# Karthik-Ragunath/RAD-NeRF

Measured on AMD Instinct MI355X. Metric: rendered frames/sec @512x512, higher is better.
Workload: dtype f32; 1 GPU; config[1]: inference 512x512, L=16 hash grid T=2^19 F=2 (xyz; ambient/torso grids tiled T=2^16 as shipped), max 16 steps/ray, 25 FPS pose stream, torso pass on; grid=hash19, engine=fused, frames_per_gpu=2122, table_dtype=f32, audio_batch=8, frames_in_flight=1, loop_launch=split, parallelism=frame-parallel x1

## Files before the change

### include/radnerf_fused.h

```cpp
#ifndef RADNERF_FUSED_H
#define RADNERF_FUSED_H

#include "radnerf_hip.h"

#ifdef __cplusplus
extern "C" {
#endif

typedef struct {
    const void *embeddings;
    const int32_t *offsets;
    uint32_t D, L, H;
    float S;
    uint32_t gridtype;
    int dtype;
} rn_grid_t;

typedef struct {
    const float *amb_w0, *amb_w1, *amb_w2;
    const float *sig_w0, *sig_w1, *sig_w2;
    const float *col_w0, *col_w1;
    uint32_t audio_dim, has_eye, ind_dim;
} rn_nerf_weights_t;

size_t rn_nerf_packed_floats(void);
size_t rn_nerf_packed_floats_h16(void);
int rn_nerf_pack_weights_h16(const rn_nerf_weights_t *w, float *packed, rn_stream_t stream);
#define RN_F32_SPLIT 2
size_t rn_nerf_packed_floats_split(void);
int rn_nerf_pack_weights_split(const rn_nerf_weights_t *w, float *packed, rn_stream_t stream);
size_t rn_nerf_bias_floats(void);
int rn_nerf_pack_weights(const rn_nerf_weights_t *w, float *packed, rn_stream_t stream);
int rn_nerf_frame_bias(const rn_nerf_weights_t *w, const float *enc_a, const float *eye, const float *ind_code,
                       float *bias, rn_stream_t stream);
int rn_nerf_frame_bias_batch(const rn_nerf_weights_t *w, const float *enc_a, uint32_t n, const float *eye, const float *ind_code,
                             float *bias, rn_stream_t stream);

int rn_nerf_fused_forward(const float *xyzs, const float *dirs, const float *deltas, uint32_t M,
                          const int32_t *m_dev, const rn_grid_t *grid_xyz, const rn_grid_t *grid_amb,
                          const float *packed, const float *bias, float bound, float *sigmas, float *rgbs,
                          float *ambient, int mlp_dtype, rn_stream_t stream);

#define RN_HEAD_STATE_INTS 64

typedef struct {
    const float *rays_o, *rays_d;
    uint32_t N;
    const float *aabb;
    float min_near;
    const uint8_t *bitfield;
    float bound, dt_gamma;
    uint32_t max_steps, cascade, grid_size;
    float T_thresh;
    float *nears, *fars;
    float *weights_sum, *depth, *image;
    int32_t *rays_alive_a, *rays_alive_b;
    float *rays_t;
    float *xyzs, *dirs, *deltas;
    float *sigmas, *rgbs;
    int32_t *state;
    uint32_t *block_counts;
    int32_t *live_slots;
    uint32_t order_w;
    const int32_t *occ_box;
} rn_head_t;

int rn_head_begin(const rn_head_t *h, rn_stream_t stream);
int rn_head_iterate(const rn_head_t *h, const rn_grid_t *grid_xyz, const rn_grid_t *grid_amb, const float *packed,
                    const float *bias, uint32_t first_iter, uint32_t n_iters, int mlp_dtype, rn_stream_t stream);
#define RN_LOOP_FIRST_MARCHED 1u
#define RN_LOOP_CLOSE_FRAME 2u
#define RN_LOOP_COOP 4u
int rn_head_iterate_ex(const rn_head_t *h, const rn_grid_t *grid_xyz, const rn_grid_t *grid_amb, const float *packed,
                       const float *bias, uint32_t first_iter, uint32_t n_iters, int mlp_dtype, uint32_t flags,
                       rn_stream_t stream);
int rn_frame_begin(const rn_head_t *h, const float *pose, float fx, float fy, float cx, float cy, uint32_t W,
                   rn_stream_t stream);
int rn_head_reschedule(const rn_head_t *h, uint32_t iter_done, uint32_t schedule_N, const int32_t *alive_total,
                       rn_stream_t stream);
#define RN_HEAD_ST_ACTIVE 4
#define RN_HEAD_ST_ITERS 16
#define RN_HEAD_ST_LIVE 17
#define RN_HEAD_ST_SLOTS 18
#define RN_HEAD_ST_UNFINISHED 19
#define RN_HEAD_ST_BARRIER 20
#define RN_HEAD_ST_STALLED 22
#define RN_HEAD_ST_HIST 32
int rn_head_check_done(const rn_head_t *h, uint32_t iters_done, rn_stream_t stream);

typedef struct {
    const float *def_w0, *def_w1, *def_w2;
    const float *tor_w0, *tor_w1, *tor_w2;
    uint32_t ind_dim;
} rn_torso_weights_t;

size_t rn_torso_packed_floats(void);
int rn_torso_pack_weights(const rn_torso_weights_t *w, float *packed, rn_stream_t stream);
int rn_torso_fused(const float *bg_coords, uint32_t N, const float *density_grid_torso, uint32_t grid_size,
                   float thresh, const float *poses6, const float *ind_code, float torso_shrink,
                   const rn_torso_weights_t *w, const float *packed, const rn_grid_t *grid_torso,
                   const float *bg_in, float *bg_out, float *torso_alpha, float *deform, rn_stream_t stream);

int rn_torso_blend_frame(const float *bg_coords, uint32_t N, const float *density_grid_torso, uint32_t grid_size,
                         float thresh, const float *poses6, const float *ind_code, float torso_shrink,
                         const rn_torso_weights_t *w, const float *packed, const rn_grid_t *grid_torso, const float *bg_in,
                         float *bg_out, float *torso_alpha, float *image, const float *weights_sum, float *depth,
                         const float *nears, const float *fars, uint8_t *image_u8, rn_stream_t stream);

#define RN_TORSO_PLAN_MAX_BYTES 268435456
size_t rn_torso_plan_bytes(uint32_t N, uint32_t n_on);
int rn_torso_plan_build(const float *bg_coords, uint32_t N, const float *density_grid_torso, uint32_t grid_size, float thresh,
                        float torso_shrink, void *plan, size_t plan_bytes, uint32_t *n_on, rn_stream_t stream);
int rn_torso_blend_frame_planned(const void *plan, size_t plan_bytes, uint32_t N, uint32_t n_on, const float *poses6,
                                 const float *ind_code, float torso_shrink, const rn_torso_weights_t *w, const float *packed,
                                 const rn_grid_t *grid_torso, const float *bg_in, float *bg_out, float *torso_alpha,
                                 float *deform, float *image, const float *weights_sum, float *depth, const float *nears,
                                 const float *fars, uint8_t *image_u8, rn_stream_t stream);

int rn_torso_mask(const float *bg_coords, uint32_t N, const float *density_grid_torso, uint32_t grid_size, float thresh,
// ... 104 lines not shown
```

### rad-nerf_amd/build.py

```python
import os
import subprocess
import sys
from concurrent.futures import ThreadPoolExecutor

ROOT = os.path.dirname(os.path.abspath(__file__))
CSRC = os.path.join(ROOT, "csrc")
LIBDIR = os.path.join(ROOT, "lib")
LIB = os.path.join(LIBDIR, "libradnerf_hip.so")
INCLUDE = os.path.join(os.path.dirname(ROOT), "include")

HIPCC = os.environ.get("HIPCC", "/opt/rocm/bin/hipcc")
ARCH = "gfx950"
CXXFLAGS = ["-O3", "-std=c++17", "-fPIC", "-ffp-contract=off", f"--offload-arch={ARCH}", "-Wall",
            "-Wno-unused-function", f"-I{INCLUDE}"]


def _sources():
    return sorted(f for f in os.listdir(CSRC) if f.endswith(".hip"))


def _headers():
    hs = [os.path.join(CSRC, f) for f in os.listdir(CSRC) if f.endswith(".h")]
    hs += [os.path.join(INCLUDE, f) for f in os.listdir(INCLUDE) if f.endswith(".h")]
    return hs


def _stale(target, deps):
    if not os.path.exists(target):
        return True
    t = os.path.getmtime(target)
    return any(os.path.getmtime(d) > t for d in deps)


def _compile(src, force):
    obj = os.path.join(CSRC, src[:-4] + ".o")
    path = os.path.join(CSRC, src)
    if force or _stale(obj, [path, __file__] + _headers()):
        cmd = [HIPCC] + CXXFLAGS + ["-c", path, "-o", obj]
        r = subprocess.run(cmd, capture_output=True, text=True)
        if r.returncode != 0:
            raise RuntimeError(f"hipcc failed for {src}:\n{r.stdout}\n{r.stderr}")
        if r.stderr.strip():
            sys.stderr.write(r.stderr)
    return obj


BINDINGS_SRC = os.path.join(CSRC, "bindings", "radnerf_pybind.cpp")
BINDINGS_DIR = os.path.join(LIBDIR, "pybind")
BINDINGS_MODULES = ("_raymarching_face", "_gridencoder", "_shencoder", "_freqencoder")


def build_bindings(force=False, verbose=False):
    import shutil
    import sysconfig
    import torch
    from torch.utils import cpp_extension as ce
    os.makedirs(BINDINGS_DIR, exist_ok=True)
    suffix = sysconfig.get_config_var("EXT_SUFFIX")
    first = os.path.join(BINDINGS_DIR, BINDINGS_MODULES[0] + suffix)
    if force or _stale(first, [BINDINGS_SRC, __file__, LIB] + _headers()):
        tlib = os.path.join(os.path.dirname(torch.__file__), "lib")
        cmd = ["g++", "-O2", "-std=c++17", "-fPIC", "-shared", "-D__HIP_PLATFORM_AMD__=1", "-DUSE_ROCM=1",
               f"-D_GLIBCXX_USE_CXX11_ABI={int(torch._C._GLIBCXX_USE_CXX11_ABI)}", "-Wno-deprecated-declarations"]
        cmd += [f"-I{p}" for p in ce.include_paths()] + [f"-I{sysconfig.get_paths()['include']}", "-I/opt/rocm/include", f"-I{INCLUDE}"]
        cmd += [BINDINGS_SRC, "-o", first, f"-L{tlib}", "-ltorch", "-ltorch_python", "-ltorch_cpu", "-lc10", "-lc10_hip",
                f"-L{LIBDIR}", "-lradnerf_hip", f"-Wl,-rpath,{tlib}", "-Wl,-rpath,$ORIGIN/.."]
        r = subprocess.run(cmd, capture_output=True, text=True)
        if r.returncode != 0:
            raise RuntimeError(f"pybind11 binding failed to build:\n{r.stdout[-3000:]}\n{r.stderr[-3000:]}")
        for name in BINDINGS_MODULES[1:]:
            shutil.copyfile(first, os.path.join(BINDINGS_DIR, name + suffix))
    if verbose:
        print(f"built {BINDINGS_DIR}/{{{', '.join(BINDINGS_MODULES)}}}{suffix}")
    return BINDINGS_DIR


def build_all(force=False, verbose=False):
    os.makedirs(LIBDIR, exist_ok=True)
    srcs = _sources()
    with ThreadPoolExecutor(max_workers=min(4, len(srcs))) as ex:
        objs = list(ex.map(lambda s: _compile(s, force), srcs))
    if force or _stale(LIB, objs):
        cmd = [HIPCC, "-shared", "-fPIC", f"--offload-arch={ARCH}", "-o", LIB] + objs
        r = subprocess.run(cmd, capture_output=True, text=True)
        if r.returncode != 0:
            raise RuntimeError(f"link failed:\n{r.stdout}\n{r.stderr}")
    if verbose:
        print(f"built {LIB}")
    return LIB


if __name__ == "__main__":
    build_all(force="--force" in sys.argv, verbose=True)
    if "--no-bindings" not in sys.argv:
        build_bindings(force="--force" in sys.argv, verbose=True)
```

### rad-nerf_amd/csrc/rn_fused.hip

```cpp
#include "rn_nerf_image_dev.h"

namespace rn {

#ifndef RN_FUSED_PAIR_HASHED
#define RN_FUSED_PAIR_HASHED 0
#endif
#ifndef RN_F32_XYZ_GROUP
#define RN_F32_XYZ_GROUP 1
#endif
#ifndef RN_F32_AMB_GROUP
#define RN_F32_AMB_GROUP 2
#endif
constexpr int kXyzGroup = RN_F32_XYZ_GROUP, kAmbGroup = RN_F32_AMB_GROUP;
#ifndef RN_F32_WAVES
#define RN_F32_WAVES 12
#endif
constexpr int kF32Waves = RN_F32_WAVES, kF32Threads = kF32Waves * kWave;
constexpr bool kPairHashed = RN_FUSED_PAIR_HASHED;

constexpr int kLdsFloats = kInferPacked + kBias;

__global__ void __launch_bounds__(256) k_pack_nerf(RawW w, float *__restrict__ packed) {
    const int e = blockIdx.x * 256 + threadIdx.x;
    if (e >= kInferPacked) return;
    packed[e] = nerf_infer_image_elem(w, e);
}

__global__ void __launch_bounds__(kBias) k_frame_bias(RawW w, const float *__restrict__ enc_a,
                                                      const float *__restrict__ eye,
                                                      const float *__restrict__ ind_code, float *__restrict__ bias) {
    const int t = threadIdx.x;
    enc_a += (size_t)blockIdx.x * w.audio_dim;
    bias += (size_t)blockIdx.x * kBias;
    bias[t] = nerf_const_bias(w, enc_a, eye, ind_code, t);
}

#ifdef RN_PHASE_CLOCK
#define RN_PHASE_MARK(i) const uint64_t phase_t##i = wall_clock64()
#define RN_PHASE_STORE()                                                                                        \
    if (p.ambient && lane < 2 && entry + 1 < M) {                                                               \
        p.ambient[2 * (size_t)sample] = (float)(lane ? phase_t3 - phase_t2 : phase_t1 - phase_t0);                \
        p.ambient[2 * (size_t)sample + 1] = (float)(lane ? phase_t4 - phase_t3 : phase_t2 - phase_t1);            \
    }
#else
#define RN_PHASE_MARK(i)
#define RN_PHASE_STORE()
#endif

template <typename TX, typename TW>
__global__ void __launch_bounds__(kF32Threads, kF32Waves / 4) k_nerf_fused(FusedParams p) {
    __shared__ __attribute__((aligned(16))) float lds[kLdsFloats];
    __shared__ LevelPlan plan_x[16], plan_w[16];

    uint32_t M = p.M;
    if (p.m_dev) { const uint32_t d = (uint32_t)*p.m_dev; M = d < M ? d : M; }
    const uint32_t n_tiles = (M + 31u) >> 5;
    if (workgroup_idle(n_tiles, kF32Waves)) return;

    for (int i = threadIdx.x; i < kInferPacked / 4; i += kF32Threads)
        reinterpret_cast<float4 *>(lds)[i] = reinterpret_cast<const float4 *>(p.packed)[i];
    if (threadIdx.x < kBias) lds[kInferPacked + threadIdx.x] = p.bias[threadIdx.x];
    if (threadIdx.x < 16) {
        const int t = threadIdx.x;
        const uint32_t ox = (uint32_t)p.gx.offsets[t], ow = (uint32_t)p.gw.offsets[t];
        plan_x[t] = plan_level<3>(p.gx.lc.scale[t], p.gx.lc.resolution[t], ox, (uint32_t)p.gx.offsets[t + 1] - ox,
                                  p.gx.gridtype, (uint32_t)sizeof(TX) * 2u);
        plan_w[t] = plan_level<2>(p.gw.lc.scale[t], p.gw.lc.resolution[t], ow, (uint32_t)p.gw.offsets[t + 1] - ow,
                                  p.gw.gridtype, (uint32_t)sizeof(TW) * 2u);
    }
    __syncthreads();

    const int lane = threadIdx.x & 63, wave = threadIdx.x >> 6;
    const int j = lane & 31, h = lane >> 5;
    const int lane_off = h * 64 + j * 2;
    const float *bias_amb = lds + kInferPacked, *bias_sig = lds + kInferPacked + 64, *bias_col = lds + kInferPacked + 128;

    const TileSchedule sched(n_tiles, kF32Waves, (uint32_t)wave);
    for (uint32_t tile = sched.first; tile < sched.end; tile += sched.stride) {
        const uint32_t entry = tile * 32 + j;
        bool live = entry < M;
        uint32_t sample = entry;
        if (p.slots) {
            if (live) sample = (uint32_t)p.slots[entry];
        } else if (live && p.deltas) {
            live = p.deltas[2 * (size_t)sample] != 0.0f;
        }
        if (__ballot(live) == 0ull) continue;

        Acc32 a0, a1, a2;
        RN_PHASE_MARK(0);
        acc_bias(a0, bias_amb, h);
        acc_bias(a2, bias_sig, h);
        {
            float in[3] = {0.0f, 0.0f, 0.0f};
            bool on = live;
            if (live) {
#pragma unroll
                for (int d = 0; d < 3; d++) {
                    in[d] = (p.xyzs[3 * (size_t)sample + d] + p.bound) / (2 * p.bound);
                    on = on && !(in[d] < 0 || in[d] > 1);
                }
            }
            LevelFetch<TX, 3, 2> f[kXyzGroup];
#pragma unroll 1
            for (int r = 0; r < 8; r += kXyzGroup) {
                if (on) {
#pragma unroll
                    for (int i = 0; i < kXyzGroup; i++)
                        issue_planned<TX, 3, 2, kPairHashed, false>(static_cast<const TX *>(p.gx.table), plan_x[2 * (r + i) + h], in, f[i]);
                }
#pragma unroll
                for (int i = 0; i < kXyzGroup; i++) {
                    float f0 = 0.0f, f1 = 0.0f;
                    if (on) {
                        TX res[2];
                        TX dummy[1];
                        blend_level<TX, 3, 2, false>(f[i], 0.0f, res, dummy);
                        f0 = to_f<TX>(res[0]);
                        f1 = to_f<TX>(res[1]);
                    }
                    step32(a0, lds + OFF_A0, 2 * (r + i), lane_off, f0);
                    step32(a2, lds + OFF_S0, 2 * (r + i), lane_off, f0);
                    step32(a0, lds + OFF_A0, 2 * (r + i) + 1, lane_off, f1);
                    step32(a2, lds + OFF_S0, 2 * (r + i) + 1, lane_off, f1);
                }
            }
        }

        RN_PHASE_MARK(1);
        acc_relu(a0);
        acc_zero(a1);
        layer_from_acc(a1, a0, lds + OFF_A1, lane_off);
        acc_relu(a1);
        float amb[2];
        valu_out<2>(a1, lds + OFF_A2, h, amb);
        amb[0] = tanhf(amb[0]);
        amb[1] = tanhf(amb[1]);
        if (p.ambient && live && h == 0) {
            p.ambient[2 * (size_t)sample] = amb[0];
            p.ambient[2 * (size_t)sample + 1] = amb[1];
        }

        RN_PHASE_MARK(2);
        {
            float in[2] = {(amb[0] + 1.0f) / 2.0f, (amb[1] + 1.0f) / 2.0f};
            const bool on = live && !(in[0] < 0 || in[0] > 1 || in[1] < 0 || in[1] > 1);
            LevelFetch<TW, 2, 2> f[kAmbGroup];
#pragma unroll 1
            for (int r = 0; r < 8; r += kAmbGroup) {
                if (on) {
#pragma unroll
                    for (int i = 0; i < kAmbGroup; i++)
                        issue_planned<TW, 2, 2, kPairHashed, false>(static_cast<const TW *>(p.gw.table), plan_w[2 * (r + i) + h], in, f[i]);
                }
#pragma unroll
                for (int i = 0; i < kAmbGroup; i++) {
                    float f0 = 0.0f, f1 = 0.0f;
                    if (on) {
                        TW res[2];
                        TW dummy[1];
                        blend_level<TW, 2, 2, false>(f[i], 0.0f, res, dummy);
                        f0 = to_f<TW>(res[0]);
                        f1 = to_f<TW>(res[1]);
                    }
                    step32(a2, lds + OFF_S0, 16 + 2 * (r + i), lane_off, f0);
                    step32(a2, lds + OFF_S0, 16 + 2 * (r + i) + 1, lane_off, f1);
                }
            }
        }

        RN_PHASE_MARK(3);
        acc_relu(a2);
        acc_zero(a1);
        layer_from_acc(a1, a2, lds + OFF_S1, lane_off);
        acc_relu(a1);
        float sigma;
        {
            float raw[1];
            valu_out<1>(a1, lds + IOFF_S2R, h, raw);
            sigma = expf(raw[0]);
        }
        if (!p.rgbs) {
            if (live && h == 0) p.sigmas[sample] = sigma;
            continue;
        }

        acc_bias(a0, bias_col, h);
        {
            float sh[16];
            float dx = 0.0f, dy = 0.0f, dz = 0.0f;
            if (live) {
                dx = p.dirs[3 * (size_t)sample]; dy = p.dirs[3 * (size_t)sample + 1]; dz = p.dirs[3 * (size_t)sample + 2];
            }
            sh_basis<4>(dx, dy, dz, sh);
#pragma unroll
            for (int s = 0; s < 8; s++) {
                const uint32_t m = 0u - (uint32_t)h;
                const uint32_t b = (__float_as_uint(sh[2 * s]) & ~m) | (__float_as_uint(sh[2 * s + 1]) & m);
                step32(a0, lds + IOFF_C0, s, lane_off, __uint_as_float(b));
            }
        }
#pragma unroll
        for (int s = 0; s < 32; s++) step32(a0, lds + IOFF_C0, 8 + s, lane_off, a1.v[s >> 4][s & 15]);
        acc_relu(a0);
        {
            float rgb[3];
            valu_out<3>(a0, lds + IOFF_C1, h, rgb);
            if (live && h == 0) {
                p.sigmas[sample] = sigma;
#pragma unroll
                for (int c = 0; c < 3; c++) p.rgbs[3 * (size_t)sample + c] = 1.0f / (1.0f + expf(-rgb[c]));
            }
        }
        RN_PHASE_MARK(4);
        RN_PHASE_STORE();
    }
}

int check_fused_grid(const rn_grid_t *g, uint32_t D, const char *name) {
    RN_REQUIRE(g && g->embeddings && g->offsets, "%s: null grid", name);
    RN_REQUIRE(g->D == D && g->L == 16, "%s: fused path needs D=%u, L=16 (got D=%u L=%u)", name, D, g->D, g->L);
    RN_REQUIRE(g->gridtype <= 1 && (g->dtype == RN_F32 || g->dtype == RN_F16), "%s: bad gridtype/dtype", name);
    RN_REQUIRE(((uintptr_t)g->embeddings & 7u) == 0, "%s: table must be 8-byte aligned", name);
    return RN_OK;
}
static int check_w(const rn_nerf_weights_t *w) {
    RN_REQUIRE(w && w->amb_w0 && w->amb_w1 && w->amb_w2 && w->sig_w0 && w->sig_w1 && w->sig_w2 && w->col_w0 && w->col_w1,
               "nerf weights: null pointer");
    RN_REQUIRE(w->has_eye <= 1 && w->audio_dim <= 1024 && w->ind_dim <= 1024, "nerf weights: bad dims");
    return RN_OK;
}

template <typename TX, typename TW>
static void launch_fused(const FusedParams &p, hipStream_t s) {
    const uint32_t n_tiles = (p.M + 31u) >> 5;
    uint32_t blocks = div_up(n_tiles, kF32Waves);
    const uint32_t cap = (uint32_t)num_cus();
    if (blocks > cap) blocks = cap;
    RN_LAUNCH_TIMED((k_nerf_fused<TX, TW>), dim3(blocks), dim3(kF32Threads), s, p);
}

int run_fused(const float *xyzs, const float *dirs, const float *deltas, uint32_t M, const int32_t *m_dev, const rn_grid_t *gx,
              const rn_grid_t *gw, const float *packed, const float *bias, float bound, float *sigmas, float *rgbs, float *ambient,
              int mlp_dtype, hipStream_t s, const int32_t *slots) {
    FusedParams p{xyzs, dirs, deltas, M, m_dev, grid_args(gx), grid_args(gw), packed, bias, bound, sigmas, rgbs, ambient, slots};
    if (mlp_dtype == RN_F32_SPLIT) {
        launch_fused_x2(p, gx->dtype, gw->dtype, (uint32_t)num_cus(), s);
    } else if (mlp_dtype == RN_F16) {
        uint32_t blocks = div_up((M + 63u) >> 6, kWavesPerBlock);
        const uint32_t cap = (uint32_t)num_cus();
        launch_fused_h16(p, gx->dtype, gw->dtype, blocks > cap ? cap : blocks, s);
    } else {
        dispatch_grid_dtypes(gx->dtype, gw->dtype, [&](auto tx, auto tw) { launch_fused<decltype(tx), decltype(tw)>(p, s); });
    }
    return RN_OK;
}

}

using namespace rn;

extern "C" {

size_t rn_nerf_packed_floats(void) { return (size_t)kInferPacked; }
size_t rn_nerf_packed_floats_h16(void) { return packed_floats_h16(); }
size_t rn_nerf_packed_floats_split(void) { return packed_floats_x2(); }

int rn_nerf_pack_weights_split(const rn_nerf_weights_t *w, float *packed, rn_stream_t stream) {
    if (int rc = check_w(w)) return rc;
    RN_REQUIRE(packed && ((uintptr_t)packed & 15u) == 0, "nerf_pack_weights_split: packed must be 16-byte aligned");
    launch_pack_nerf_x2(raw_w(w), packed, as_stream(stream));
    return check_launch("nerf_pack_weights_split");
}

int rn_nerf_pack_weights_h16(const rn_nerf_weights_t *w, float *packed, rn_stream_t stream) {
    if (int rc = check_w(w)) return rc;
    RN_REQUIRE(packed && ((uintptr_t)packed & 15u) == 0, "nerf_pack_weights_h16: packed must be 16-byte aligned");
    launch_pack_nerf_h16(raw_w(w), packed, as_stream(stream));
    return check_launch("nerf_pack_weights_h16");
}
size_t rn_nerf_bias_floats(void) { return (size_t)kBias; }

int rn_nerf_pack_weights(const rn_nerf_weights_t *w, float *packed, rn_stream_t stream) {
    if (int rc = check_w(w)) return rc;
    RN_REQUIRE(packed && ((uintptr_t)packed & 15u) == 0, "nerf_pack_weights: packed must be 16-byte aligned");
    hipLaunchKernelGGL(k_pack_nerf, dim3(div_up(kInferPacked, 256)), dim3(256), 0, as_stream(stream), raw_w(w), packed);
    return check_launch("nerf_pack_weights");
}

int rn_nerf_frame_bias(const rn_nerf_weights_t *w, const float *enc_a, const float *eye, const float *ind_code,
                       float *bias, rn_stream_t stream) {
    if (int rc = check_w(w)) return rc;
    RN_REQUIRE(bias, "nerf_frame_bias: null output");
    RN_REQUIRE(enc_a || w->audio_dim == 0, "nerf_frame_bias: enc_a is required");
    RN_REQUIRE(eye || !w->has_eye, "nerf_frame_bias: eye is required when has_eye");
    RN_REQUIRE(ind_code || w->ind_dim == 0, "nerf_frame_bias: ind_code is required when ind_dim > 0");
    hipLaunchKernelGGL(k_frame_bias, dim3(1), dim3(kBias), 0, as_stream(stream), raw_w(w), enc_a, eye, ind_code, bias);
    return check_launch("nerf_frame_bias");
}

int rn_nerf_frame_bias_batch(const rn_nerf_weights_t *w, const float *enc_a, uint32_t n, const float *eye, const float *ind_code,
                             float *bias, rn_stream_t stream) {
    if (n == 0) return RN_OK;
    if (int rc = check_w(w)) return rc;
    RN_REQUIRE(bias && (enc_a || w->audio_dim == 0) && (eye || !w->has_eye) && (ind_code || w->ind_dim == 0),
               "nerf_frame_bias_batch: null pointer");
    hipLaunchKernelGGL(k_frame_bias, dim3(n), dim3(kBias), 0, as_stream(stream), raw_w(w), enc_a, eye, ind_code, bias);
    return check_launch("nerf_frame_bias_batch");
}

int rn_nerf_fused_forward(const float *xyzs, const float *dirs, const float *deltas, uint32_t M, const int32_t *m_dev,
                          const rn_grid_t *grid_xyz, const rn_grid_t *grid_amb, const float *packed, const float *bias,
                          float bound, float *sigmas, float *rgbs, float *ambient, int mlp_dtype, rn_stream_t stream) {
    if (M == 0) return RN_OK;
    RN_REQUIRE(xyzs && packed && bias && sigmas && (dirs || !rgbs), "nerf_fused_forward: null pointer");
    RN_REQUIRE(((uintptr_t)packed & 15u) == 0, "nerf_fused_forward: packed must be 16-byte aligned");
    if (int rc = check_fused_grid(grid_xyz, 3, "nerf_fused_forward(xyz grid)")) return rc;
    if (int rc = check_fused_grid(grid_amb, 2, "nerf_fused_forward(ambient grid)")) return rc;
    RN_REQUIRE(mlp_dtype == RN_F32 || mlp_dtype == RN_F16 || mlp_dtype == RN_F32_SPLIT,
               "nerf_fused_forward: mlp_dtype must be RN_F32, RN_F16 or RN_F32_SPLIT");
    run_fused(xyzs, dirs, deltas, M, m_dev, grid_xyz, grid_amb, packed, bias, bound, sigmas, rgbs, ambient, mlp_dtype,
              as_stream(stream));
    return check_launch("nerf_fused_forward");
}

}
```

### rad-nerf_amd/csrc/rn_fused_dev.h

```cpp
#pragma once

#include "rn_dda_dev.h"
#include "rn_grid_dev.h"
#include "rn_sh_dev.h"
#include "rn_tile32_dev.h"

#include "../../include/radnerf_fused.h"

#ifndef RN_XCD_TILES
#define RN_XCD_TILES 1
#endif
#ifndef RN_TILE_CHUNK
#define RN_TILE_CHUNK 2
#endif

namespace rn {

constexpr int kFusedThreads = 512;
constexpr int kWavesPerBlock = kFusedThreads / kWave;

struct RawW {
    const float *amb_w0, *amb_w1, *amb_w2, *sig_w0, *sig_w1, *sig_w2, *col_w0, *col_w1;
    uint32_t audio_dim, has_eye, ind_dim;
};
inline RawW raw_w(const rn_nerf_weights_t *w) {
    return RawW{w->amb_w0, w->amb_w1, w->amb_w2, w->sig_w0, w->sig_w1, w->sig_w2, w->col_w0, w->col_w1,
                w->audio_dim, w->has_eye, w->ind_dim};
}

struct Acc {
    f32x16 v[2][2];
};

__device__ __forceinline__ void acc_zero(Acc &a) {
#pragma unroll
    for (int nt = 0; nt < 2; nt++)
#pragma unroll
        for (int rt = 0; rt < 2; rt++)
#pragma unroll
            for (int r = 0; r < 16; r++) a.v[nt][rt][r] = 0.0f;
}

__device__ __forceinline__ void acc_bias(Acc &a, const float *bias64, int h) {
#pragma unroll
    for (int rt = 0; rt < 2; rt++)
#pragma unroll
        for (int g = 0; g < 4; g++) {
            const float4 b = *reinterpret_cast<const float4 *>(bias64 + 32 * rt + 8 * g + 4 * h);
            a.v[0][rt][4 * g + 0] = b.x; a.v[0][rt][4 * g + 1] = b.y; a.v[0][rt][4 * g + 2] = b.z; a.v[0][rt][4 * g + 3] = b.w;
            a.v[1][rt][4 * g + 0] = b.x; a.v[1][rt][4 * g + 1] = b.y; a.v[1][rt][4 * g + 2] = b.z; a.v[1][rt][4 * g + 3] = b.w;
        }
}

__device__ __forceinline__ void acc_relu(Acc &a) {
#pragma unroll
    for (int nt = 0; nt < 2; nt++)
#pragma unroll
        for (int rt = 0; rt < 2; rt++)
#pragma unroll
            for (int r = 0; r < 16; r++) a.v[nt][rt][r] = relu_bits(a.v[nt][rt][r]);
}


template <int NOUT>
__device__ __forceinline__ void valu_out(const Acc &in, const float *wl, int h, float (&part)[2][NOUT]) {
#pragma unroll
    for (int o = 0; o < NOUT; o++) {
        float p0 = 0.0f, p1 = 0.0f;
        const float *wo = wl + (o * 2 + h) * 32;
#pragma unroll
        for (int g = 0; g < 8; g++) {
            const float4 w = *reinterpret_cast<const float4 *>(wo + 4 * g);
            const int rt = g >> 2, r = (g & 3) * 4;
            p0 = __builtin_fmaf(in.v[0][rt][r + 0], w.x, p0); p1 = __builtin_fmaf(in.v[1][rt][r + 0], w.x, p1);
            p0 = __builtin_fmaf(in.v[0][rt][r + 1], w.y, p0); p1 = __builtin_fmaf(in.v[1][rt][r + 1], w.y, p1);
            p0 = __builtin_fmaf(in.v[0][rt][r + 2], w.z, p0); p1 = __builtin_fmaf(in.v[1][rt][r + 2], w.z, p1);
            p0 = __builtin_fmaf(in.v[0][rt][r + 3], w.w, p0); p1 = __builtin_fmaf(in.v[1][rt][r + 3], w.w, p1);
        }
        part[0][o] = p0 + __shfl_xor(p0, 32, 64);
        part[1][o] = p1 + __shfl_xor(p1, 32, 64);
    }
}


struct GridArgs {
    const void *table;
    const int32_t *offsets;
    LevelConsts lc;
    uint32_t gridtype;
};
inline GridArgs grid_args(const rn_grid_t *g) {
    return GridArgs{g->embeddings, g->offsets, make_level_consts(g->L, g->S, g->H), g->gridtype};
}

struct FusedParams {
    const float *xyzs, *dirs, *deltas;
    uint32_t M;
    const int32_t *m_dev;
    GridArgs gx, gw;
    const float *packed, *bias;
    float bound;
    float *sigmas, *rgbs, *ambient;
    const int32_t *slots;
};

struct TileSchedule {
    uint32_t first, end, stride;
    __device__ __forceinline__ TileSchedule(uint32_t n_tiles, uint32_t waves_per_block, uint32_t wave) {
        const uint32_t G = gridDim.x, b = blockIdx.x;
#if RN_XCD_TILES
        if (G >= 8 && (G & 7u) == 0) {
            const uint32_t xcd = b & 7u, local = b >> 3, per_xcd = (n_tiles + 7u) >> 3;
            const uint32_t lo = xcd * per_xcd, hi = lo + per_xcd < n_tiles ? lo + per_xcd : n_tiles;
            constexpr uint32_t C = RN_TILE_CHUNK;
            const uint32_t chunk = (C < waves_per_block && waves_per_block % C == 0) ? C : waves_per_block, B = G >> 3;
            first = lo + ((wave / chunk) * B + local) * chunk + wave % chunk;
            end = lo < hi ? hi : lo;
            stride = B * waves_per_block;
            return;
        }
#endif
        first = b * waves_per_block + wave;
        end = n_tiles;
        stride = G * waves_per_block;
    }
};


__device__ __forceinline__ uint32_t launch_samples(uint32_t M, const int32_t *m_dev) {
    if (m_dev) { const uint32_t d = (uint32_t)*m_dev; M = d < M ? d : M; }
    return M;
}

__device__ __forceinline__ uint32_t live_count(uint32_t M, const int32_t *m_dev) {
    if (!m_dev) return M;
    const int32_t d = *m_dev;
    return d <= 0 ? 0u : ((uint32_t)d < M ? (uint32_t)d : M);
}

__device__ __forceinline__ bool workgroup_idle(uint32_t n_tiles, uint32_t waves_per_block) {
    const TileSchedule w0(n_tiles, waves_per_block, 0u);
    return w0.first >= w0.end;
}

__device__ __forceinline__ bool entry_slot(const int32_t *slots, const float *deltas, uint32_t entry, uint32_t M, uint32_t &sample) {
    bool live = entry < M;
    sample = entry;
    if (slots) {
        if (live) sample = (uint32_t)slots[entry];
    } else if (live && deltas) {
        live = deltas[2 * (size_t)sample] != 0.0f;
    }
    return live;
}

__device__ __forceinline__ void load_dir(const float *dirs, bool live, uint32_t sample, float &dx, float &dy, float &dz) {
    if (live && dirs) {
        dx = dirs[3 * (size_t)sample]; dy = dirs[3 * (size_t)sample + 1]; dz = dirs[3 * (size_t)sample + 2];
    }
}

template <typename F>
static inline void dispatch_grid_dtypes(int gx_dtype, int gw_dtype, F &&f) {
    if (gx_dtype == RN_F32 && gw_dtype == RN_F32) f(float{}, float{});
    else if (gx_dtype == RN_F16 && gw_dtype == RN_F16) f(__half{}, __half{});
    else if (gx_dtype == RN_F32) f(float{}, __half{});
    else f(__half{}, float{});
}

static inline int check_train_grid(const rn_grid_t *g, uint32_t D, const char *what) {
    RN_REQUIRE(g && g->embeddings && g->offsets, "%s grid is null", what);
    RN_REQUIRE(g->D == D && g->L == 16 && g->dtype == RN_F32, "%s grid must be D=%u, L=16, fp32 with C=2", what, D);
    return RN_OK;
}

int check_fused_grid(const rn_grid_t *g, uint32_t D, const char *name);
int run_fused(const float *xyzs, const float *dirs, const float *deltas, uint32_t M, const int32_t *m_dev, const rn_grid_t *gx,
              const rn_grid_t *gw, const float *packed, const float *bias, float bound, float *sigmas, float *rgbs, float *ambient,
              int mlp_dtype, hipStream_t s, const int32_t *slots = nullptr);
void launch_fused_h16(const FusedParams &p, int gx_dtype, int gw_dtype, uint32_t blocks, hipStream_t s);
void launch_pack_nerf_h16(const RawW &w, float *packed, hipStream_t s);
size_t packed_floats_h16();
void launch_fused_x2(const FusedParams &p, int gx_dtype, int gw_dtype, uint32_t n_cus, hipStream_t s);
void launch_pack_nerf_x2(const RawW &w, float *packed, hipStream_t s);
size_t packed_floats_x2();

}
```

### rad-nerf_amd/radnerf_hip/abi.py

```python
import ctypes as C

_int, _u32, _f32, _f64, _sz, _ptr, _P = C.c_int, C.c_uint32, C.c_float, C.c_double, C.c_size_t, C.c_void_p, C.POINTER
_i64 = C.c_int64

RN_F32, RN_F16 = 0, 1
RN_LAYOUT_LBC, RN_LAYOUT_BLC, RN_LAYOUT_BLC_LEVELMAJOR = 0, 1, 2

RN_F32_SPLIT = 2
RN_HEAD_STATE_INTS = 64
RN_TORSO_PLAN_MAX_BYTES = 256 << 20
RN_LOOP_FIRST_MARCHED, RN_LOOP_CLOSE_FRAME, RN_LOOP_COOP = 1, 2, 4
RN_HEAD_ST_ACTIVE, RN_HEAD_ST_ITERS, RN_HEAD_ST_LIVE, RN_HEAD_ST_SLOTS = 4, 16, 17, 18
RN_HEAD_ST_UNFINISHED, RN_HEAD_ST_STALLED, RN_HEAD_ST_HIST = 19, 22, 32


class GridT(C.Structure):
    c_name = "rn_grid_t"
    _fields_ = [("embeddings", _ptr), ("offsets", _ptr), ("D", _u32), ("L", _u32), ("H", _u32), ("S", _f32),
                ("gridtype", _u32), ("dtype", _int)]


class NerfWeightsT(C.Structure):
    c_name = "rn_nerf_weights_t"
    _fields_ = [("amb_w0", _ptr), ("amb_w1", _ptr), ("amb_w2", _ptr), ("sig_w0", _ptr), ("sig_w1", _ptr),
# ... 38 lines not shown
class HeadGradsT(C.Structure):
    c_name = "rn_train_head_grads_t"
    _fields_ = [(n, _ptr) for n in ("amb_w0", "amb_w1", "amb_w2", "sig_w0", "sig_w1", "sig_w2", "col_w0", "col_w1",
                                    "enc_a", "eye", "ind_code")]


class ScatterJobT(C.Structure):
    c_name = "rn_scatter_job_t"
    _fields_ = [("grad", _ptr), ("inputs", _ptr), ("grid", _P(GridT)), ("offsets_host", _ptr), ("grad_table", _ptr)]


class TorsoGradsT(C.Structure):
    c_name = "rn_train_torso_grads_t"
    _fields_ = [(n, _ptr) for n in ("def_w0", "def_w1", "def_w2", "tor_w0", "tor_w1", "tor_w2", "ind_code")]


class TrainSetT(C.Structure):
    c_name = "rn_train_set_t"
    _fields_ = [("images", _ptr), ("torso", _ptr), ("bg", _ptr), ("poses", _ptr), ("face_rect", _ptr), ("eye", _ptr),
                ("auds", _ptr), ("fx", _f32), ("fy", _f32), ("cx", _f32), ("cy", _f32), ("H", _u32), ("W", _u32), ("F", _u32),
                ("Fa", _u32), ("C", _u32), ("att", _u32), ("torso_mode", _u32)]


class SchedTensorT(C.Structure):
    c_name = "rn_sched_tensor_t"
    _fields_ = [("param", _ptr), ("grad", _ptr), ("exp_avg", _ptr), ("exp_avg_sq", _ptr), ("shadow", _ptr), ("numel", _u32),
                ("lr0", _f32)]


FUNCTIONS = {
    "rn_last_error": (C.c_char_p, []),
    "rn_version": (_int, []),
    "rn_device_count": (_int, []),
    "rn_prof_enable": (_int, [_int]),
    "rn_prof_pause": (_int, [_int]),
    "rn_prof_collect": (_int, [C.POINTER(_u32), C.POINTER(_f32)]),
    "rn_prof_durations": (_int, [C.POINTER(_f32), _u32]),
    "rn_near_far_from_aabb": (_int, [_ptr, _ptr, _ptr, _u32, _f32, _ptr, _ptr, _ptr]),
    "rn_sph_from_ray": (_int, [_ptr, _ptr, _f32, _u32, _ptr, _ptr]),
    "rn_morton3D": (_int, [_ptr, _u32, _ptr, _ptr]),
    "rn_morton3D_invert": (_int, [_ptr, _u32, _ptr, _ptr]),
    "rn_packbits": (_int, [_ptr, _u32, _f32, _ptr, _ptr]),
    "rn_morton3D_dilation": (_int, [_ptr, _u32, _u32, _ptr, _ptr]),
    "rn_march_rays_train_workspace": (_sz, [_u32]),
    "rn_march_rays_train": (_int, [_ptr, _ptr, _ptr, _f32, _f32, _u32, _u32, _u32, _u32, _u32, _ptr, _ptr, _ptr, _ptr, _ptr,
                                   _ptr, _ptr, _ptr, _ptr, _ptr]),
    "rn_march_rays_train_budget": (_int, [_ptr, _ptr, _ptr, _f32, _f32, _u32, _u32, _u32, _u32, _u32, _ptr, _ptr, _ptr, _ptr,
                                          _ptr, _ptr, _ptr, _ptr, _ptr, _ptr, _ptr]),
    "rn_march_rays_train_step_state": (_sz, [_u32]),
    "rn_march_rays_train_step": (_int, [_ptr, _ptr, _ptr, _ptr, _f32, _f32, _f32, _u32, _u32, _u32, _u32, _u32, _ptr, _ptr,
                                        _ptr, _ptr, _ptr, _ptr, _ptr, _ptr, _ptr, _ptr, _u32, _ptr]),
    "rn_march_rays_train_backward": (_int, [_ptr, _ptr, _ptr, _ptr, _u32, _u32, _ptr, _ptr, _ptr]),
    "rn_composite_rays_train_forward": (_int, [_ptr, _ptr, _ptr, _ptr, _ptr, _u32, _u32, _f32, _ptr, _ptr, _ptr, _ptr, _ptr]),
    "rn_composite_rays_train_backward": (_int, [_ptr, _ptr, _ptr, _ptr, _ptr, _ptr, _ptr, _ptr, _ptr, _ptr, _ptr, _u32, _u32,
                                                _f32, _ptr, _ptr, _ptr, _ptr]),
    "rn_march_rays": (_int, [_u32, _u32, _ptr, _ptr, _ptr, _ptr, _f32, _f32, _u32, _u32, _u32, _ptr, _ptr, _ptr, _ptr, _ptr,
                             _ptr, _ptr, _ptr, _ptr]),
    "rn_composite_rays": (_int, [_u32, _u32, _f32, _ptr, _ptr, _ptr, _ptr, _ptr, _ptr, _ptr, _ptr, _ptr, _ptr]),
    "rn_compact_rays_workspace": (_sz, [_u32]),
    "rn_compact_rays": (_int, [_ptr, _u32, _ptr, _ptr, _ptr, _ptr, _ptr]),
    "rn_grid_encode_forward": (_int, [_ptr, _ptr, _ptr, _ptr, _u32, _u32, _u32, _u32, _f32, _u32, _ptr, _u32, _int, _u32, _int,
                                      _int, _ptr]),
    "rn_grid_encode_forward_workspace": (_sz, [_u32, _u32, _u32, _int]),
    "rn_grid_encode_forward_ws": (_int, [_ptr, _ptr, _ptr, _ptr, _ptr, _u32, _u32, _u32, _u32, _f32, _u32, _ptr, _u32, _int,
                                         _u32, _int, _int, _ptr, _sz, _ptr]),
    "rn_grid_encode_forward_bound": (_int, [_ptr, _f32, _ptr, _ptr, _ptr, _ptr, _u32, _u32, _u32, _u32, _f32, _u32, _u32, _int,
                                            _int, _ptr, _sz, _ptr]),
    "rn_grid_encode_backward": (_int, [_ptr, _ptr, _ptr, _ptr, _ptr, _u32, _u32, _u32, _u32, _f32, _u32, _ptr, _ptr, _u32, _int,
                                       _u32, _int, _int, _ptr]),
    "rn_grad_total_variation": (_int, [_ptr, _ptr, _ptr, _ptr, _f32, _u32, _u32, _u32, _u32, _f32, _u32, _u32, _int, _ptr]),
    "rn_sh_encode_forward": (_int, [_ptr, _ptr, _u32, _u32, _u32, _ptr, _ptr]),
    "rn_sh_encode_backward": (_int, [_ptr, _ptr, _u32, _u32, _u32, _ptr, _ptr, _ptr]),
    "rn_freq_encode_forward": (_int, [_ptr, _u32, _u32, _u32, _u32, _ptr, _ptr]),
    "rn_freq_encode_backward": (_int, [_ptr, _ptr, _u32, _u32, _u32, _u32, _ptr, _ptr]),
    "rn_nerf_packed_floats": (_sz, []),
    "rn_nerf_packed_floats_h16": (_sz, []),
    "rn_nerf_pack_weights_h16": (_int, [_P(NerfWeightsT), _ptr, _ptr]),
    "rn_nerf_packed_floats_split": (_sz, []),
    "rn_nerf_pack_weights_split": (_int, [_P(NerfWeightsT), _ptr, _ptr]),
    "rn_nerf_bias_floats": (_sz, []),
    "rn_nerf_pack_weights": (_int, [_P(NerfWeightsT), _ptr, _ptr]),
    "rn_nerf_frame_bias": (_int, [_P(NerfWeightsT), _ptr, _ptr, _ptr, _ptr, _ptr]),
    "rn_nerf_frame_bias_batch": (_int, [_P(NerfWeightsT), _ptr, _u32, _ptr, _ptr, _ptr, _ptr]),
    "rn_nerf_fused_forward": (_int, [_ptr, _ptr, _ptr, _u32, _ptr, _P(GridT), _P(GridT), _ptr, _ptr, _f32, _ptr, _ptr, _ptr,
                                     _int, _ptr]),
    "rn_head_begin": (_int, [_P(HeadT), _ptr]),
    "rn_head_iterate": (_int, [_P(HeadT), _P(GridT), _P(GridT), _ptr, _ptr, _u32, _u32, _int, _ptr]),
    "rn_head_iterate_ex": (_int, [_P(HeadT), _P(GridT), _P(GridT), _ptr, _ptr, _u32, _u32, _int, _u32, _ptr]),
    "rn_frame_begin": (_int, [_P(HeadT), _ptr, _f32, _f32, _f32, _f32, _u32, _ptr]),
    "rn_head_reschedule": (_int, [_P(HeadT), _u32, _u32, _ptr, _ptr]),
    "rn_head_check_done": (_int, [_P(HeadT), _u32, _ptr]),
    "rn_torso_packed_floats": (_sz, []),
    "rn_torso_pack_weights": (_int, [_P(TorsoWeightsT), _ptr, _ptr]),
    "rn_torso_fused": (_int, [_ptr, _u32, _ptr, _u32, _f32, _ptr, _ptr, _f32, _P(TorsoWeightsT), _ptr, _P(GridT), _ptr, _ptr,
                              _ptr, _ptr, _ptr]),
    "rn_torso_blend_frame": (_int, [_ptr, _u32, _ptr, _u32, _f32, _ptr, _ptr, _f32, _P(TorsoWeightsT), _ptr, _P(GridT), _ptr,
                                    _ptr, _ptr, _ptr, _ptr, _ptr, _ptr, _ptr, _ptr, _ptr]),
    "rn_torso_plan_bytes": (_sz, [_u32, _u32]),
    "rn_torso_plan_build": (_int, [_ptr, _u32, _ptr, _u32, _f32, _f32, _ptr, _sz, C.POINTER(_u32), _ptr]),
    "rn_torso_blend_frame_planned": (_int, [_ptr, _sz, _u32, _u32, _ptr, _ptr, _f32, _P(TorsoWeightsT), _ptr, _P(GridT), _ptr, _ptr,
                                            _ptr, _ptr, _ptr, _ptr, _ptr, _ptr, _ptr, _ptr, _ptr]),
    "rn_torso_mask": (_int, [_ptr, _u32, _ptr, _u32, _f32, _ptr, _ptr]),
    "rn_blend_frame": (_int, [_ptr, _ptr, _ptr, _ptr, _ptr, _ptr, _u32, _ptr, _ptr]),
    "rn_occupancy_workspace": (_sz, [_u32, _u32]),
    "rn_occupancy_points": (_int, [_u32, _u32, _f32, _ptr, _u32, _ptr, _ptr]),
    "rn_occupancy_update": (_int, [_ptr, _f32, _ptr, _u32, _u32, _f32, _f32, _ptr, _ptr, _ptr, _ptr]),
    "rn_mark_untrained_grid": (_int, [_ptr, _u32, _u32, _f64, _f64, _f64, _f64, _u32, _u32, _f32, _ptr, _ptr]),
    "rn_torso_grid_points": (_int, [_u32, _ptr, _u32, _ptr, _ptr]),
    "rn_torso_grid_update": (_int, [_ptr, _ptr, _u32, _f32, _ptr, _ptr]),
    "rn_occ_box": (_int, [_ptr, _u32, _u32, _ptr, _ptr]),
    "rn_hash_u01_bits": (_u32, [_u32, _u32]),
    "rn_audio_encode_windows": (_int, [_P(AudioWeightsT), _ptr, _u32, _ptr, _ptr, _ptr]),
    "rn_audio_encode_windows_backward": (_int, [_P(AudioWeightsT), _ptr, _u32, _ptr, _ptr, _P(AudioGradsT), _ptr, _ptr]),
    "rn_audio_train_acts_floats": (_sz, [_u32, _int]),
    "rn_audio_encode_windows_train": (_int, [_P(AudioWeightsT), _ptr, _u32, _ptr, _ptr, _ptr, _ptr]),
    "rn_audio_encode_windows_backward_acts": (_int, [_P(AudioWeightsT), _ptr, _u32, _ptr, _ptr, _P(AudioGradsT), _ptr, _ptr,
                                                     _ptr]),
    "rn_audio_backward_partials_floats": (_sz, [_u32, _int]),
    "rn_audio_encode_windows_backward_ordered": (_int, [_P(AudioWeightsT), _ptr, _u32, _ptr, _ptr, _P(AudioGradsT), _ptr, _ptr,
                                                        _ptr, _ptr]),
    "rn_audio_encode_stream": (_int, [_P(AudioWeightsT), _ptr, _u32, _u32, _u32, _ptr, _ptr, _ptr]),
    "rn_audio_smooth": (_int, [_ptr, _u32, _u32, _f32, _ptr, _int, _ptr]),
    "rn_audio_smooth_seq": (_int, [_ptr, _u32, _u32, _f32, _ptr, _int, _ptr, _ptr]),
    "rn_get_rays": (_int, [_ptr, _f32, _f32, _f32, _f32, _u32, _u32, _ptr, _ptr, _ptr]),
    "rn_get_bg_coords": (_int, [_u32, _u32, _ptr, _ptr]),
    "rn_convert_poses": (_int, [_ptr, _u32, _ptr, _ptr]),
    "rn_mlp64_image_floats": (_sz, [_u32, _u32, _u32]),
    "rn_mlp64_tile_floats": (_sz, [_u32]),
    "rn_mlp64_wgrad_workspace": (_sz, [_u32]),
    "rn_mlp64_pack": (_int, [_ptr, _u32, _ptr, _ptr, _u32, _u32, _u32, _ptr, _ptr]),
    "rn_mlp64_forward": (_int, [_ptr, _u32, _ptr, _ptr, _u32, _u32, _u32, _ptr, _ptr, _ptr, _ptr]),
    "rn_mlp64_backward": (_int, [_ptr, _u32, _ptr, _u32, _u32, _u32, _ptr, _ptr, _ptr, _ptr, _ptr, _ptr]),
    "rn_mlp64_weight_grads": (_int, [_ptr, _ptr, _u32, _u32, _u32, _u32, _ptr, _ptr, _ptr, _ptr, _ptr, _u32, _ptr, _ptr, _ptr,
                                     _ptr, _ptr]),
    "rn_head_mid_forward": (_int, [_ptr, _ptr, _u32, _u32, _ptr, _ptr, _ptr]),
    "rn_head_mid_backward": (_int, [_ptr, _ptr, _ptr, _u32, _u32, _ptr, _ptr]),
    "rn_abs_sum2_forward": (_int, [_ptr, _u32, _ptr, _ptr]),
    "rn_abs_sum2_backward": (_int, [_ptr, _ptr, _u32, _ptr, _ptr]),
    "rn_train_loss": (_int, [_ptr, _ptr, _ptr, _ptr, _ptr, _ptr, _u32, _ptr, _ptr, _ptr, _ptr, _ptr]),
    "rn_adam_step": (_int, [_P(AdamTensorT), _u32, _f32, _f32, _f32, _ptr, _ptr, _ptr]),
    "rn_adam_step_lr": (_int, [_P(AdamTensorT), _u32, _f32, _f32, _f32, _ptr, _ptr, _ptr, _ptr]),
    "rn_mesh_workspace": (_sz, [_u32, _u32, _u32]),
    "rn_mesh_lattice_points": (_int, [_u32, _u32, _u32, _ptr, _u32, _u32, _ptr, _ptr]),
    "rn_mesh_count": (_int, [_ptr, _u32, _u32, _u32, _f32, _ptr, _ptr, _ptr]),
    "rn_mesh_emit": (_int, [_ptr, _u32, _u32, _u32, _f32, _ptr, _ptr, _u32, _u32, _ptr, _ptr, _ptr]),
    "rn_mesh_tet_case": (_int, [_u32, _P(C.c_int32), _P(C.c_int32)]),
    "rn_train_head_image_floats": (_sz, []),
    "rn_train_head_workspace_floats": (_sz, [_u32]),
    "rn_train_head_wgrad_workspace": (_sz, []),
    "rn_train_head_pack": (_int, [_P(NerfWeightsT), _ptr, _ptr, _ptr, _ptr, _ptr]),
    "rn_train_head_pack_row": (_int, [_P(NerfWeightsT), _ptr, _ptr, _ptr, _ptr, _ptr, _ptr]),
    "rn_train_head_forward": (_int, [_ptr, _ptr, _u32, _ptr, _P(GridT), _P(GridT), _ptr, _f32, _ptr, _ptr, _ptr, _ptr, _ptr,
                                     _ptr, _ptr, _ptr]),
    "rn_train_head_backward": (_int, [_ptr, _ptr, _ptr, _ptr, _ptr, _ptr, _u32, _ptr, _ptr, _ptr, _ptr, _ptr, _ptr]),
    "rn_train_head_input_grads": (_int, [_ptr, _ptr, _ptr, _u32, _ptr, _P(GridT), _ptr, _ptr, _f32, _ptr, _ptr, _ptr]),
    "rn_train_head_weight_grads": (_int, [_P(NerfWeightsT), _ptr, _ptr, _ptr, _u32, _ptr, _ptr, _P(HeadGradsT), _ptr, _ptr]),
    "rn_train_head_weight_grads_row": (_int, [_P(NerfWeightsT), _ptr, _ptr, _ptr, _ptr, _u32, _u32, _ptr, _ptr, _P(HeadGradsT),
                                              _ptr, _ptr]),
    "rn_train_head_image_floats_h16": (_sz, []),
    "rn_train_head_pack_h16": (_int, [_P(NerfWeightsT), _ptr, _ptr, _ptr, _ptr, _ptr]),
    "rn_train_head_pack_row_h16": (_int, [_P(NerfWeightsT), _ptr, _ptr, _ptr, _ptr, _ptr, _ptr]),
    "rn_train_head_forward_h16": (_int, [_ptr, _ptr, _u32, _ptr, _P(GridT), _P(GridT), _ptr, _f32, _ptr, _ptr, _ptr, _ptr, _ptr,
                                         _ptr, _ptr, _ptr]),
    "rn_train_head_backward_h16": (_int, [_ptr, _ptr, _ptr, _ptr, _ptr, _ptr, _u32, _ptr, _ptr, _ptr, _ptr, _ptr, _ptr]),
    "rn_grid_scatter_lbc": (_int, [_ptr, _ptr, _u32, _ptr, _P(GridT), _ptr, _ptr]),
    "rn_grid_scatter_workspace": (_sz, [_u32, _P(GridT), _ptr]),
# ... 48 lines not shown
```

Before: 1322 frames/s.

## Split fused NeRF activations across half-waves and use exact reciprocal bound

Several micro-optimizations go into the fused NeRF inference kernel. When the bound is a power of two, the per-sample divide by 2*bound becomes a multiply by an exactly computed reciprocal. The tanh, exp and sigmoid activations and the output stores are split between the two half-waves, so each lane does fewer transcendentals and the stores are spread out. The shared-memory plans and weights are placed in one aligned struct, and the file is compiled with SLP vectorization disabled. Together these reduce ALU work in the epilogue but add a cross-lane shuffle and more divergent store paths.

```diff
diff --git a/include/radnerf_fused.h b/include/radnerf_fused.h
--- a/include/radnerf_fused.h
+++ b/include/radnerf_fused.h
@@ -35,6 +35,7 @@
                        float *bias, rn_stream_t stream);
 int rn_nerf_frame_bias_batch(const rn_nerf_weights_t *w, const float *enc_a, uint32_t n, const float *eye, const float *ind_code,
                              float *bias, rn_stream_t stream);
+int rn_nerf_bound_rcp_exact(float bound);
 
 int rn_nerf_fused_forward(const float *xyzs, const float *dirs, const float *deltas, uint32_t M,
                           const int32_t *m_dev, const rn_grid_t *grid_xyz, const rn_grid_t *grid_amb,
diff --git a/rad-nerf_amd/build.py b/rad-nerf_amd/build.py
--- a/rad-nerf_amd/build.py
+++ b/rad-nerf_amd/build.py
@@ -13,6 +13,11 @@
 ARCH = "gfx950"
 CXXFLAGS = ["-O3", "-std=c++17", "-fPIC", "-ffp-contract=off", f"--offload-arch={ARCH}", "-Wall",
             "-Wno-unused-function", f"-I{INCLUDE}"]
+FILE_FLAGS = {"rn_fused.hip": ["-fno-slp-vectorize"]}
+
+
+def flags_for(src):
+    return CXXFLAGS + FILE_FLAGS.get(src, [])
 
 
 def _sources():
@@ -36,7 +41,7 @@
     obj = os.path.join(CSRC, src[:-4] + ".o")
     path = os.path.join(CSRC, src)
     if force or _stale(obj, [path, __file__] + _headers()):
-        cmd = [HIPCC] + CXXFLAGS + ["-c", path, "-o", obj]
+        cmd = [HIPCC] + flags_for(src) + ["-c", path, "-o", obj]
         r = subprocess.run(cmd, capture_output=True, text=True)
         if r.returncode != 0:
             raise RuntimeError(f"hipcc failed for {src}:\n{r.stdout}\n{r.stderr}")
diff --git a/rad-nerf_amd/csrc/rn_fused.hip b/rad-nerf_amd/csrc/rn_fused.hip
--- a/rad-nerf_amd/csrc/rn_fused.hip
+++ b/rad-nerf_amd/csrc/rn_fused.hip
@@ -17,6 +17,15 @@
 #endif
 constexpr int kF32Waves = RN_F32_WAVES, kF32Threads = kF32Waves * kWave;
 constexpr bool kPairHashed = RN_FUSED_PAIR_HASHED;
+#ifndef RN_F32_RCP_BOUND
+#define RN_F32_RCP_BOUND 1
+#endif
+#ifndef RN_F32_PLANS_FIRST
+#define RN_F32_PLANS_FIRST 1
+#endif
+#ifndef RN_F32_HALF_ACT
+#define RN_F32_HALF_ACT 1
+#endif
 
 constexpr int kLdsFloats = kInferPacked + kBias;
 
@@ -49,8 +58,17 @@
 
 template <typename TX, typename TW>
 __global__ void __launch_bounds__(kF32Threads, kF32Waves / 4) k_nerf_fused(FusedParams p) {
+#if RN_F32_PLANS_FIRST
+    __shared__ struct __attribute__((aligned(16))) {
+        LevelPlan plan_x[16], plan_w[16];
+        float lds[kLdsFloats];
+    } sm;
+    LevelPlan (&plan_x)[16] = sm.plan_x, (&plan_w)[16] = sm.plan_w;
+    float *const lds = sm.lds;
+#else
     __shared__ __attribute__((aligned(16))) float lds[kLdsFloats];
     __shared__ LevelPlan plan_x[16], plan_w[16];
+#endif
 
     uint32_t M = p.M;
     if (p.m_dev) { const uint32_t d = (uint32_t)*p.m_dev; M = d < M ? d : M; }
@@ -74,6 +92,10 @@
     const int j = lane & 31, h = lane >> 5;
     const int lane_off = h * 64 + j * 2;
     const float *bias_amb = lds + kInferPacked, *bias_sig = lds + kInferPacked + 64, *bias_col = lds + kInferPacked + 128;
+#if RN_F32_RCP_BOUND
+    float inv_2bound;
+    const bool rcp_bound = bound_rcp_exact(p.bound, &inv_2bound);
+#endif
 
     const TileSchedule sched(n_tiles, kF32Waves, (uint32_t)wave);
     for (uint32_t tile = sched.first; tile < sched.end; tile += sched.stride) {
@@ -96,10 +118,19 @@
             bool on = live;
             if (live) {
 #pragma unroll
-                for (int d = 0; d < 3; d++) {
-                    in[d] = (p.xyzs[3 * (size_t)sample + d] + p.bound) / (2 * p.bound);
-                    on = on && !(in[d] < 0 || in[d] > 1);
-                }
+                for (int d = 0; d < 3; d++) in[d] = p.xyzs[3 * (size_t)sample + d] + p.bound;
+#if RN_F32_RCP_BOUND
+                if (rcp_bound) {
+#pragma unroll
+                    for (int d = 0; d < 3; d++) in[d] = in[d] * inv_2bound;
+                } else
+#endif
+                {
+#pragma unroll
+                    for (int d = 0; d < 3; d++) in[d] = in[d] / (2 * p.bound);
+                }
+#pragma unroll
+                for (int d = 0; d < 3; d++) on = on && !(in[d] < 0 || in[d] > 1);
             }
             LevelFetch<TX, 3, 2> f[kXyzGroup];
 #pragma unroll 1
@@ -134,12 +165,22 @@
         acc_relu(a1);
         float amb[2];
         valu_out<2>(a1, lds + OFF_A2, h, amb);
+#if RN_F32_HALF_ACT
+        {
+            const float mine = tanhf(h ? amb[1] : amb[0]);
+            const float other = __shfl_xor(mine, 32, 64);
+            if (p.ambient && live) p.ambient[2 * (size_t)sample + h] = mine;
+            amb[0] = h ? other : mine;
+            amb[1] = h ? mine : other;
+        }
+#else
         amb[0] = tanhf(amb[0]);
         amb[1] = tanhf(amb[1]);
         if (p.ambient && live && h == 0) {
             p.ambient[2 * (size_t)sample] = amb[0];
             p.ambient[2 * (size_t)sample + 1] = amb[1];
         }
+#endif
 
         RN_PHASE_MARK(2);
         {
@@ -174,6 +215,15 @@
         acc_zero(a1);
         layer_from_acc(a1, a2, lds + OFF_S1, lane_off);
         acc_relu(a1);
+#if RN_F32_HALF_ACT
+        float raw[1];
+        valu_out<1>(a1, lds + IOFF_S2R, h, raw);
+        if (!p.rgbs) {
+            const float sigma = expf(raw[0]);
+            if (live && h == 1) p.sigmas[sample] = sigma;
+            continue;
+        }
+#else
         float sigma;
         {
             float raw[1];
@@ -184,6 +234,7 @@
             if (live && h == 0) p.sigmas[sample] = sigma;
             continue;
         }
+#endif
 
         acc_bias(a0, bias_col, h);
         {
@@ -206,11 +257,22 @@
         {
             float rgb[3];
             valu_out<3>(a0, lds + IOFF_C1, h, rgb);
+#if RN_F32_HALF_ACT
+            const float e0 = expf(h ? -rgb[2] : -rgb[0]);
+            const float e1 = expf(h ? raw[0] : -rgb[1]);
+            const float s0 = 1.0f / (1.0f + e0), s1 = 1.0f / (1.0f + e1);
+            if (live) {
+                float *const rgb_out = p.rgbs + 3 * (size_t)sample;
+                rgb_out[2 * h] = s0;
+                *(h ? p.sigmas + sample : rgb_out + 1) = h ? e1 : s1;
+            }
+#else
             if (live && h == 0) {
                 p.sigmas[sample] = sigma;
 #pragma unroll
                 for (int c = 0; c < 3; c++) p.rgbs[3 * (size_t)sample + c] = 1.0f / (1.0f + expf(-rgb[c]));
             }
+#endif
         }
         RN_PHASE_MARK(4);
         RN_PHASE_STORE();
@@ -309,6 +371,11 @@
     return check_launch("nerf_frame_bias_batch");
 }
 
+int rn_nerf_bound_rcp_exact(float bound) {
+    float inv;
+    return bound_rcp_exact(bound, &inv) ? 1 : 0;
+}
+
 int rn_nerf_fused_forward(const float *xyzs, const float *dirs, const float *deltas, uint32_t M, const int32_t *m_dev,
                           const rn_grid_t *grid_xyz, const rn_grid_t *grid_amb, const float *packed, const float *bias,
                           float bound, float *sigmas, float *rgbs, float *ambient, int mlp_dtype, rn_stream_t stream) {
diff --git a/rad-nerf_amd/csrc/rn_fused_dev.h b/rad-nerf_amd/csrc/rn_fused_dev.h
--- a/rad-nerf_amd/csrc/rn_fused_dev.h
+++ b/rad-nerf_amd/csrc/rn_fused_dev.h
@@ -104,6 +104,13 @@
     const int32_t *slots;
 };
 
+__host__ __device__ inline bool bound_rcp_exact(float bound, float *inv) {
+    const uint32_t b = __builtin_bit_cast(uint32_t, bound);
+    const bool ok = (b & 0x807fffffu) == 0u && b >= 0x00800000u && b <= 0x7d800000u;
+    *inv = __builtin_bit_cast(float, ok ? 0x7e800000u - b : 0u);
+    return ok;
+}
+
 struct TileSchedule {
     uint32_t first, end, stride;
     __device__ __forceinline__ TileSchedule(uint32_t n_tiles, uint32_t waves_per_block, uint32_t wave) {
diff --git a/rad-nerf_amd/radnerf_hip/abi.py b/rad-nerf_amd/radnerf_hip/abi.py
--- a/rad-nerf_amd/radnerf_hip/abi.py
+++ b/rad-nerf_amd/radnerf_hip/abi.py
@@ -144,6 +144,7 @@
     "rn_nerf_pack_weights": (_int, [_P(NerfWeightsT), _ptr, _ptr]),
     "rn_nerf_frame_bias": (_int, [_P(NerfWeightsT), _ptr, _ptr, _ptr, _ptr, _ptr]),
     "rn_nerf_frame_bias_batch": (_int, [_P(NerfWeightsT), _ptr, _u32, _ptr, _ptr, _ptr, _ptr]),
+    "rn_nerf_bound_rcp_exact": (_int, [_f32]),
     "rn_nerf_fused_forward": (_int, [_ptr, _ptr, _ptr, _u32, _ptr, _P(GridT), _P(GridT), _ptr, _ptr, _f32, _ptr, _ptr, _ptr,
                                      _int, _ptr]),
     "rn_head_begin": (_int, [_P(HeadT), _ptr]),
```

Result: slower. 1292 frames/s (-2.2%).
